# WangYuTum/odometry

Hardware: AMD Instinct MI355X
Metric: tracked frames/sec (1241x376, 4-level pyramid) (higher is better)
Workload: dtype f32

## Files before the change

odometry_amd/csrc/kernels.hip.h:

```cpp
#pragma once
#include <hip/hip_runtime.h>
#include "odo_math.h"

#ifndef ODO_PHASE_STAMPS
#define ODO_PHASE_STAMPS 0
#endif
#if ODO_PHASE_STAMPS
#define ODO_DBG(a) ((a).dbg)
#else
#define ODO_DBG(a) ((unsigned long long*)nullptr)
#endif

#ifndef ODO_KERNEL
#define ODO_KERNEL __global__
#define ODO_KERNEL_T __global__
#endif
#ifdef ODO_LM_CHAIN_TU
#define ODO_DEVICE_VAR static __device__
#else
#define ODO_DEVICE_VAR __device__
#endif

namespace odo {

// ... 425 lines not shown
  }
  for (int x0 = 4; x0 < cols - 4; x0 += 256) {
    const int x = x0 + t;
    float d = 0.0f;
    const bool f = (x < cols - 4) && depth_valid(d = D[x]);
    const unsigned long long bal = __ballot(f);
    const int pre = __popcll(bal & ((1ull << lane) - 1ull));
    if (lane == 0) wave_tot[wv] = __popcll(bal);
    __syncthreads();
    int off = base_sh;
    for (int w = 0; w < wv; w++) off += wave_tot[w];
    if (f) {
      const PointK p = make_point(x, y, d, I[x], k);
      const int i = off + pre;
      pl.a[i] = make_float4(p.X, p.Y, p.Z, p.i1);
      pl.b[i] = make_float4(p.fx_z, p.jw02, p.jw03, p.jw04);
      pl.c[i] = make_float4(p.jw05, p.jw12, p.jw13, p.jw14);
      pl.d[i] = p.jw15;
    }
    __syncthreads();
    if (t == 0) base_sh += (wave_tot[0] + wave_tot[1]) + (wave_tot[2] + wave_tot[3]);
    __syncthreads();
  }
  if (t == 0 && (int)blockIdx.x == kl.row_base[l + 1] - 1) npts[l] = base_sh;
}
ODO_KERNEL void __launch_bounds__(256) kf_fill_kernel(KfLevels kl, float f0, float cx0, float cy0,
                                                      const int* __restrict__ rowcnt, int* __restrict__ npts, PointList pl0, PointList pl1,
                                                      PointList pl2, PointList pl3, PointList pl4, PointList pl5,
                                                      PointList pl6, PointList pl7, int dense_above) {
  const int l = kf_find_level(kl, blockIdx.x);
  const PointList pl = l == 0 ? pl0 : l == 1 ? pl1 : l == 2 ? pl2 : l == 3 ? pl3 : l == 4 ? pl4 : l == 5 ? pl5 : l == 6 ? pl6 : pl7;
  kf_fill_kernel_body<KfLevels>(kl, l, pl, f0, cx0, cy0, rowcnt, npts, dense_above);
}

__device__ __forceinline__ PointK load_point(const PointList& pl, int i) {
  const float4 a = pl.a[i], b = pl.b[i], c = pl.c[i];
  PointK p;
  p.X = a.x; p.Y = a.y; p.Z = a.z; p.i1 = a.w;
  p.fx_z = b.x; p.jw02 = b.y; p.jw03 = b.z; p.jw04 = b.w;
  p.jw05 = c.x; p.jw12 = c.y; p.jw13 = c.z; p.jw14 = c.w;
  p.jw15 = pl.d[i];
  return p;
}

__device__ __forceinline__ const float* lm_uniform_ptr(const float* p) {
  const unsigned long long v = (unsigned long long)p;
  const unsigned lo = (unsigned)__builtin_amdgcn_readfirstlane((int)(v & 0xffffffffu)), hi = (unsigned)__builtin_amdgcn_readfirstlane((int)(v >> 32));
  return (const float*)(((unsigned long long)hi << 32) | lo);
}
__device__ __forceinline__ float ldg_f32(const float* base_uniform, unsigned byte_off) {
  typedef __attribute__((address_space(1))) const char GlobalBytes;
  typedef __attribute__((address_space(1))) const float GlobalFloat;
  return *(GlobalFloat*)((GlobalBytes*)base_uniform + byte_off);
}
template <bool kMayBilinear>
__device__ __forceinline__ bool point_residual_g(const PointK& p, const float* T, const LevelK& k, const float* I2_uniform, int rows,
                                                 int cols, float* r, float J[6]) {
  if (kMayBilinear && k.bilinear) return point_residual<true>(p, T, k, I2_uniform, rows, cols, r, J);
  const float t0 = ((T[0] * p.X + T[4] * p.Y) + T[8] * p.Z) + T[12];
  const float t1 = ((T[1] * p.X + T[5] * p.Y) + T[9] * p.Z) + T[13];
  const float t2 = ((T[2] * p.X + T[6] * p.Y) + T[10] * p.Z) + T[14];
  if (!(t2 > 0.0f)) return false;
  const double t2d = (double)t2, y = rcp_refined_d(t2d);
  const float u = (float)(div_shared_d(k.fl * (double)t0, t2d, y) + (double)k.cx);
  const float v = (float)(div_shared_d(k.fl * (double)t1, t2d, y) + (double)k.cy);
  const float fu = floorf(u), fv = floorf(v);
  if (!(fu < (float)cols) || !(fv < (float)rows) || !(fu >= 0.0f) || !(fv >= 0.0f)) return false;
  const int ui = (int)fu, vi = (int)fv;
  const int px = (ui - 1 >= 0) ? ui - 1 : 0, nx = (ui + 1 < cols) ? ui + 1 : cols - 1;
  const int py = (vi - 1 >= 0) ? vi - 1 : 0, ny = (vi + 1 < rows) ? vi + 1 : rows - 1;
  const unsigned row = (unsigned)vi * (unsigned)cols, ucols = (unsigned)cols;
  const float tc = ldg_f32(I2_uniform, (row + (unsigned)ui) * 4u), tl = ldg_f32(I2_uniform, (row + (unsigned)px) * 4u),
              tr = ldg_f32(I2_uniform, (row + (unsigned)nx) * 4u), tu = ldg_f32(I2_uniform, ((unsigned)py * ucols + (unsigned)ui) * 4u),
              td = ldg_f32(I2_uniform, ((unsigned)ny * ucols + (unsigned)ui) * 4u);
  const float gx = 0.5f * (tr - tl), gy = 0.5f * (td - tu);
  *r = tc - p.i1;
  J[0] = gx * p.fx_z;
  J[1] = gy * p.fx_z;
  J[2] = gx * p.jw02 + gy * p.jw12;
  J[3] = gx * p.jw03 + gy * p.jw13;
  J[4] = gx * p.jw04 + gy * p.jw14;
  J[5] = gx * p.jw05 + gy * p.jw15;
  return true;
}

ODO_KERNEL void __launch_bounds__(kLmBlock) lm_residual_list_kernel(PointList pl, int n, const float* __restrict__ I2, int rows,
                                                                     int cols, LevelK k, const LmState* __restrict__ st,
                                                                     int expect_level, int robust, float huber_delta,
                                                                     const float* __restrict__ scale_sqr_ptr,
                                                                     double* __restrict__ partials) {
  if (!(st->active != 0 && st->level == expect_level)) return;
  float T[16];
#pragma unroll
  for (int i = 0; i < 16; i++) T[i] = st->T[i];
  const float scale_sqr = (robust == 2) ? *scale_sqr_ptr : 1.0f;
  double acc[ODO_NACC];
#pragma unroll
  for (int q = 0; q < ODO_NACC; q++) acc[q] = 0.0;
  for (int idx = blockIdx.x * kLmBlock + threadIdx.x; idx < n; idx += gridDim.x * kLmBlock) {
    const PointK p = load_point(pl, idx);
    float r, J[6];
    if (!point_residual(p, T, k, I2, rows, cols, &r, J)) continue;
    const float w = robust_weight(r, robust, huber_delta, scale_sqr);
    accumulate_row(acc, r, w, J);
  }
  block_reduce_acc(acc, partials + (size_t)blockIdx.x * ODO_NACC);
}

ODO_KERNEL void __launch_bounds__(kLmBlock) lm_residual_only_list_kernel(PointList pl, int n, const float* __restrict__ I2,
                                                                          int rows, int cols, LevelK k,
                                                                          const LmState* __restrict__ st, int expect_level,
                                                                          float* __restrict__ res) {
  if (!(st->active != 0 && st->level == expect_level)) return;
  float T[16];
#pragma unroll
  for (int i = 0; i < 16; i++) T[i] = st->T[i];
  for (int idx = blockIdx.x * kLmBlock + threadIdx.x; idx < n; idx += gridDim.x * kLmBlock) {
    const PointK p = load_point(pl, idx);
    float r = __builtin_nanf(""), rr;
    if (point_residual_only(p, T, k, I2, rows, cols, &rr)) r = rr;
    res[idx] = r;
  }
}

ODO_KERNEL void __launch_bounds__(kLmBlock) lm_residual_only_kernel(LevelView v, LevelK k, const LmState* __restrict__ st,
                                                                     int expect_level, float* __restrict__ res) {
  if (!(st->active != 0 && st->level == expect_level)) return;
  float T[16];
#pragma unroll
  for (int i = 0; i < 16; i++) T[i] = st->T[i];
  const int iw = v.cols - 8, ih = v.rows - 8;
  const int n = (iw > 0 && ih > 0) ? iw * ih : 0;
  for (int idx = blockIdx.x * kLmBlock + threadIdx.x; idx < n; idx += gridDim.x * kLmBlock) {
    const int y = 4 + idx / iw, x = 4 + idx % iw;
    const size_t o = (size_t)y * v.cols + x;
    const float d = v.D1[o];
    float r = __builtin_nanf("");
    if (depth_valid(d)) {
      const PointK p = make_point(x, y, d, v.I1[o], k);
      float rr;
      if (point_residual_only(p, T, k, v.I2, v.rows, v.cols, &rr)) r = rr;
    }
    res[idx] = r;
  }
}

static_assert(sizeof(LmState) <= 64 * sizeof(int), "LmState must fit one wavefront-wide copy");
static_assert(sizeof(LmState) == 64 * sizeof(int), "LmState is exactly 64 dwords");

struct LmTraceRow {
  int level, iter, n_res, accepted, stop;
  float err, lambda_after;
  float delta[6];
};
constexpr int kTraceCap = 128;

__device__ __forceinline__ double readlane_d(double v, int src_lane) {
  const int lo = __builtin_amdgcn_readlane(__double2loint(v), src_lane);
  const int hi = __builtin_amdgcn_readlane(__double2hiint(v), src_lane);
  return __hiloint2double(hi, lo);
}

__device__ __forceinline__ void solve_damped_wave_regs(const double* acc, float lambda, float delta_out[6]) {
  const int lane = threadIdx.x & 63;
  const int i = lane >> 3, j = lane & 7;
  const bool in = (i < 6 && j < 7);
// ... 112 lines not shown
    for (int i = 0; i < 9; i++) {
      const float id = (i == 0 || i == 4 || i == 8) ? 1.0f : 0.0f;
      V[i] = (id + ca * Om[i]) + cb * Om2[i];
    }
  }
  o->tx = (V[0] * a[0] + V[1] * a[1]) + V[2] * a[2];
  o->ty = (V[3] * a[0] + V[4] * a[1]) + V[5] * a[2];
  o->tz = (V[6] * a[0] + V[7] * a[1]) + V[8] * a[2];
}
__device__ __forceinline__ void lm_apply_step_wave(LmState* s, int max_iters) {
  Se3 d;
  se3_exp_wave(s->delta, &d);
  se3_left_update(d, s->cur, &s->inc);
  se3_to_colmajor(s->inc, s->T);
  s->iter++;
  if (!(max_iters > s->iter)) { s->active = 0; s->stop_reason = 3; }
}

constexpr int kRowFloats = 15;
constexpr int kRowSub = 8;
template <int T> struct RowBuf {
  static constexpr int kStride = T / kRowSub + 4;
  static constexpr int W = kRowSub * kStride;
  static constexpr int kBytes = kRowFloats * W * (int)sizeof(float);
};

__device__ __forceinline__ void rows_store(float* __restrict__ rows, int W, int t, const float J[6], float w, float r, bool valid) {
  const int p = (t % kRowSub) * (W / kRowSub) + t / kRowSub;
#pragma unroll
  for (int a = 0; a < 6; a++) {
    rows[a * W + p] = valid ? J[a] : 0.0f;
    rows[(6 + a) * W + p] = valid ? J[a] * w : 0.0f;
  }
  rows[12 * W + p] = valid ? r : 0.0f;
  rows[13 * W + p] = valid ? r * w : 0.0f;
  rows[14 * W + p] = valid ? 1.0f : 0.0f;
}
__device__ __forceinline__ void rows_store_z(float* __restrict__ rows, int W, int t, const float J[6], float w, float r, bool valid) {
  const int p = (t % kRowSub) * (W / kRowSub) + t / kRowSub;
#pragma unroll
  for (int a = 0; a < 6; a++) {
    rows[a * W + p] = J[a];
    rows[(6 + a) * W + p] = J[a] * w;
  }
  rows[12 * W + p] = r;
  rows[13 * W + p] = r * w;
  rows[14 * W + p] = valid ? 1.0f : 0.0f;
}
__device__ __forceinline__ void rows_of_quantity(int q, int* rowA, int* rowB) {
  int a = 0, k = q;
  while (a < 5 && k >= 6 - a) { k -= 6 - a; a++; }
  if (q < 21) { *rowA = 6 + a; *rowB = a + k; }
  else if (q < 27) { *rowA = 6 + (q - 21); *rowB = 12; }
  else if (q == 27) { *rowA = 13; *rowB = 12; }
  else { *rowA = 14; *rowB = 14; }
}
template <int CTRL> __device__ __forceinline__ double dpp_d(double v) {
  const int lo = __builtin_amdgcn_update_dpp(0, __double2loint(v), CTRL, 0xf, 0xf, false);
  const int hi = __builtin_amdgcn_update_dpp(0, __double2hiint(v), CTRL, 0xf, 0xf, false);
  return __hiloint2double(hi, lo);
}
__device__ __forceinline__ double rows_butterfly8(double acc) {
  const double up = dpp_d<0x104>(acc), dn = dpp_d<0x114>(acc);
  acc += (threadIdx.x & 4) ? dn : up;
  acc += dpp_d<0x4E>(acc);
  acc += dpp_d<0xB1>(acc);
  return acc;
}
template <int T, int S>
__device__ __forceinline__ double rows_accumulate(const float* __restrict__ rows, int rowA, int rowB, int s, double acc) {
  static_assert(S == kRowSub && (T / S) % 4 == 0, "the row layout is built for S sub-lanes");
  constexpr int W = RowBuf<T>::W;
  const float4* A = (const float4*)(rows + rowA * W + s * RowBuf<T>::kStride);
  const float4* B = (const float4*)(rows + rowB * W + s * RowBuf<T>::kStride);
#pragma unroll
  for (int i = 0; i < T / S / 4; i++) {
    const float4 a = A[i], b = B[i];
    acc = fma((double)a.x, (double)b.x, acc);
    acc = fma((double)a.y, (double)b.y, acc);
    acc = fma((double)a.z, (double)b.z, acc);
    acc = fma((double)a.w, (double)b.w, acc);
  }
  return acc;
}

__device__ __forceinline__ double wave_sum64(double v) {
  v += dpp_d<0xB1>(v);
  v += dpp_d<0x4E>(v);
  v += dpp_d<0x141>(v);
  v += dpp_d<0x140>(v);
  const double r0 = readlane_d(v, 0), r1 = readlane_d(v, 16), r2 = readlane_d(v, 32), r3 = readlane_d(v, 48);
  return (r0 + r1) + (r2 + r3);
}
__device__ __forceinline__ float tdist_term(float e2, float sigma_sqr) { return e2 * (1.0f + 200.0f) / (200.0f + e2 / sigma_sqr); }
__device__ __forceinline__ float tdist_next_sigma(double total, int n) { return sqrtf((float)(total / (double)n)); }
__device__ __forceinline__ bool tdist_converged(float nxt, float cur) { return !(fabsf(nxt - cur) >= 1e-3f); }
constexpr int kTdistMaxPasses = 1000;

constexpr int kTdistChunksMax = 640;
ODO_KERNEL void __launch_bounds__(1024) lm_tdist_scale_kernel(const float* __restrict__ res, int n,
                                                               const LmState* __restrict__ st, int expect_level,
                                                               float* __restrict__ scale_sqr_out, int list_order,
                                                               int* __restrict__ only_if = nullptr) {
  if (!(st->active != 0 && st->level == expect_level)) return;
  if (only_if) {
    if (__hip_atomic_load(only_if, __ATOMIC_RELAXED, __HIP_MEMORY_SCOPE_AGENT) == 0) return;
    __syncthreads();
    if (threadIdx.x == 0) {
      __hip_atomic_store(only_if, 0, __ATOMIC_RELAXED, __HIP_MEMORY_SCOPE_AGENT);
      only_if[1] += 1;
    }
  }
  __shared__ double shs[1024];
  __shared__ int shn[1024];
  __shared__ float sh_sigma;
  __shared__ int sh_done;
  const int t = threadIdx.x;
  float cur = 5.0f;
  if (list_order) {
    double* part = shs;
    const int lane = t & 63, wv = t >> 6;
    const int nchunk = (n + 63) / 64;
    int n_valid = 0;
    constexpr int kPer = kTdistChunksMax / 16;
    float e2[kPer];
    int cnt = 0;
#pragma unroll
    for (int u = 0; u < kPer; u++) {
      const int c = wv + 16 * u, i = 64 * c + lane;
      const float r = (c < nchunk && i < n) ? res[i] : __builtin_nanf("");
      const bool ok = (r == r);
      e2[u] = ok ? r * r : -1.0f;
      cnt += __popcll(__ballot(ok));
    }
    for (int pass = 0; pass < kTdistMaxPasses; pass++) {
      const float sigma_sqr = cur * cur;
#pragma unroll
      for (int u = 0; u < kPer; u++) {
        const int c = wv + 16 * u;
        if (c < nchunk) {
          const double ws = wave_sum64(e2[u] >= 0.0f ? (double)tdist_term(e2[u], sigma_sqr) : 0.0);
          if (lane == 0) part[c] = ws;
        }
      }
      if (pass == 0 && lane == 0) shn[wv] = cnt;
      __syncthreads();
      if (pass == 0) {
        int tot = 0;
#pragma unroll
        for (int w = 0; w < 16; w++) tot += shn[w];
        n_valid = tot;
      }
      double a = 0.0;
      for (int v = lane; 4 * v < nchunk; v += 64) {
        const int c = 4 * v;
        const double p1 = (c + 1 < nchunk) ? part[c + 1] : 0.0, p2 = (c + 2 < nchunk) ? part[c + 2] : 0.0, p3 = (c + 3 < nchunk) ? part[c + 3] : 0.0;
        a += ((part[c] + p1) + p2) + p3;
      }
      const double total = wave_sum64(a);
      const float nxt = (n_valid > 0) ? tdist_next_sigma(total, n_valid) : cur;
      const bool done = (n_valid == 0) || tdist_converged(nxt, cur);
      cur = nxt;
      if (done) break;
      __syncthreads();
    }
    if (t == 0) *scale_sqr_out = cur * cur;
// ... 489 lines not shown
                                                 const ChainOut chain = ChainOut{nullptr, nullptr, 0, 0, 0, 0, 0, 0, 0, 0}) {
  const int t = threadIdx.x;
  if (t < 64) {
    if (t < (int)(sizeof(LmState) / sizeof(int))) ((int*)st_out)[t] = ((const int*)&s_sh)[t];
    if (final_state && s_sh.finished && t < (int)(sizeof(LmState) / sizeof(int))) ((int*)final_state)[t] = ((const int*)&s_sh)[t];
    if (t == 0) {
      if (s_sh.finished && out) lm_write_result(s_sh, cost_stat, out, done_flag, token, chain);
      if (host_prog) {
        if (s_sh.finished) __hip_atomic_store(host_prog + 1, token, __ATOMIC_RELAXED, __HIP_MEMORY_SCOPE_SYSTEM);
        __hip_atomic_store(host_prog, (token << kProgSeqBits) | (seq + 1), __ATOMIC_RELEASE, __HIP_MEMORY_SCOPE_SYSTEM);
      }
    }
  }
}

__device__ __forceinline__ void lm_step_body(const StepArgs& a, const StepLaunch& q) {
  if (lm_chain_skip(a)) return;
  __builtin_amdgcn_s_setprio(3);
  lm_span_begin(q.span);
  __shared__ LmState s_sh;
  __shared__ double fold_sh[8 * 32];
  __shared__ double acc_sh[32];
  const bool publisher = (blockIdx.x == gridDim.x - 1);
  if (ODO_DBG(a) && publisher && threadIdx.x == 0 && q.seq < 56) ODO_DBG(a)[16 + 2 * q.seq] = wall_clock64();
  lm_fused_prologue(q.st_in, q.part_in, a.lv, a.n_levels, a.lambda0, a.precision, s_sh, fold_sh, acc_sh, a.trace, a.cost_stat,
                    publisher, q.first_of_solve ? a.init : nullptr, a.stop_level);
  const bool run = (s_sh.active != 0 && s_sh.status == 0);
  const int lvl = run ? s_sh.level : 0;
  const StepLevel& L = a.lv[lvl];
  if (run && !publisher && (int)blockIdx.x < L.nblk) {
    __shared__ float rows_sh[kRowFloats * RowBuf<kLmBlock>::W];
    constexpr int kS = 8;
    const int my_q = threadIdx.x / kS, my_s = threadIdx.x % kS;
    int rowA = 0, rowB = 0;
    if (my_q < ODO_NACC) rows_of_quantity(my_q, &rowA, &rowB);
    float T[16];
#pragma unroll
    for (int i = 0; i < 16; i++) T[i] = s_sh.T[i];
    double accq = 0.0;
    const int first = blockIdx.x * kLmBlock;
    for (int base = first; base < L.n; base += L.nblk * kLmBlock) {
      const int idx = base + threadIdx.x;
      float r = 0.0f, w = 0.0f, J[6] = {0.0f, 0.0f, 0.0f, 0.0f, 0.0f, 0.0f};
      bool valid = false;
      if (idx < L.n) {
        const PointK p = load_point(L.pl, idx);
        if (point_residual(p, T, L.k, L.I2, L.rows, L.cols, &r, J)) {
          w = robust_weight(r, a.robust, a.huber_delta, 1.0f);
          valid = true;
        }
      }
      if (base > first) __syncthreads();
      rows_store(rows_sh, RowBuf<kLmBlock>::W, threadIdx.x, J, w, r, valid);
      __syncthreads();
      if (my_q < ODO_NACC) accq = rows_accumulate<kLmBlock, kS>(rows_sh, rowA, rowB, my_s, accq);
    }
    accq = rows_butterfly8(accq);
    if (my_q < ODO_NACC && my_s == 0) q.part_out[(size_t)blockIdx.x * ODO_NACC + my_q] = accq;
  }
  if (publisher) {
    if (threadIdx.x == 0 && run) { s_sh.pending = 1; s_sh.pending_nblk = L.nblk; }
    __syncthreads();
    lm_fused_publish(s_sh, q.st_out, a.host_prog, q.seq, a.token, a.cost_stat, a.out, a.done_flag, a.final_state, chain_out_of(a));
    if (ODO_DBG(a) && threadIdx.x == 0 && q.seq < 56) ODO_DBG(a)[16 + 2 * q.seq + 1] = wall_clock64();
  }
  lm_span_end(q.span);
}

ODO_KERNEL void __launch_bounds__(kLmBlock) lm_step_kernel(StepArgs a) {
  const StepLaunch q = {a.st_in, a.st_out, a.part_in, a.part_out, a.seq, a.first_of_solve, a.span};
  lm_step_body(a, q);
}
ODO_KERNEL void __launch_bounds__(kLmBlock) lm_step_kernel_batch(const StepArgs* __restrict__ table, int seq, int first_of_solve,
                                                                 unsigned long long* span) {
  const StepArgs& a = table[blockIdx.y];
  const StepLaunch q = {a.st2[seq & 1], a.st2[(seq + 1) & 1], a.part2[seq & 1], a.part2[(seq + 1) & 1], seq, first_of_solve, span};
  lm_step_body(a, q);
}

#ifndef ODO_COARSE_BLOCK
#define ODO_COARSE_BLOCK 512
#endif
constexpr int kCoarseBlock = ODO_COARSE_BLOCK;
constexpr int kCoarseLdsBytes = 2 * RowBuf<kLmBlock>::kBytes;
constexpr int kCoarseMaxPoints = 1024;

constexpr int kCoarseRounds = kCoarseMaxPoints / kCoarseBlock;
constexpr int kCoarseChunks = kCoarseRounds * (kCoarseBlock / kWave);
__device__ __forceinline__ float coarse_tdist_sigma(double (*part)[kCoarseChunks], int* cnt, const float e2[kCoarseRounds],
                                                    const bool valid[kCoarseRounds], int nr) {
  constexpr int kW = kCoarseBlock / kWave;
  const int lane = threadIdx.x & 63, wv = threadIdx.x >> 6;
  int my_cnt[kCoarseRounds];
#pragma unroll
  for (int rd = 0; rd < kCoarseRounds; rd++) my_cnt[rd] = __popcll(__ballot(rd < nr && valid[rd]));
  float sigma = 5.0f;
  int n_total = 0;
  for (int pass = 0; pass < kTdistMaxPasses; pass++) {
#pragma unroll
    for (int rd = 0; rd < kCoarseRounds; rd++) {
      const double ws = wave_sum64((rd < nr && valid[rd]) ? (double)tdist_term(e2[rd], sigma * sigma) : 0.0);
      if (lane == 0) { part[pass & 1][rd * kW + wv] = ws; if (pass == 0) cnt[rd * kW + wv] = my_cnt[rd]; }
    }
    __syncthreads();
    if (pass == 0) {
      int tot = 0;
#pragma unroll
      for (int i = 0; i < kCoarseChunks; i++) tot += cnt[i];
      n_total = tot;
    }
    double G = 0.0;
    if (lane < kCoarseChunks / 4) {
      const double* pv = &part[pass & 1][(lane >> 1) * kW + 4 * (lane & 1)];
      G = ((pv[0] + pv[1]) + pv[2]) + pv[3];
    }
    const double total = wave_sum64(G);
    const float nxt = (n_total > 0) ? tdist_next_sigma(total, n_total) : sigma;
    const bool done = (n_total == 0) || tdist_converged(nxt, sigma);
    sigma = nxt;
    if (done) break;
  }
  return sigma;
}
#if ODO_PHASE_STAMPS
ODO_DEVICE_VAR unsigned long long g_lm_diag[24];
#endif
constexpr unsigned long long kArmWaitTicks = 200000000ull;
template <bool kFull, bool kArmed = false>
__device__ __forceinline__ void lm_coarse_body(const StepArgs& a, const StepLaunch& q, int min_level, const unsigned* __restrict__ lv_src) {
#if ODO_PHASE_STAMPS
  const unsigned long long w_entry = (unsigned long long)wall_clock64();
#endif
  if (!kArmed && lm_chain_skip(a)) return;
  __builtin_amdgcn_s_setprio(3);
  lm_span_begin(q.span);
  __shared__ LmState s_sh;
  extern __shared__ __attribute__((aligned(16))) double red_sh[];
  __shared__ double acc_sh[32];
  __shared__ StepLevel lv_sh[ODO_MAX_LEVELS_K];
  __shared__ unsigned long long sm_sh[4];
  unsigned long long arm_g0 = 0;
  if (kArmed && threadIdx.x < 17) arm_g0 = __hip_atomic_load(a.arm + threadIdx.x, __ATOMIC_RELAXED, __HIP_MEMORY_SCOPE_SYSTEM);
  lm_copy_levels(lv_sh, lv_src);
  if (threadIdx.x == 0) {
#pragma unroll
    for (int i = 0; i < 4; i++) sm_sh[i] = 0;
  }
  __shared__ __attribute__((aligned(16))) float arm_pose_sh[16];
  __shared__ __attribute__((aligned(16))) int arm_verdict_sh4[4];
  if (kArmed) {
    if (threadIdx.x < 64) {
      const int lane = (int)threadIdx.x;
      unsigned long long g = arm_g0;
      bool got = __all(lane >= 17 || (int)(g >> 32) == a.token);
      const unsigned long long t0 = (unsigned long long)wall_clock64();
      for (int spin = 0; !got; spin++) {
        if (lane < 17) g = __hip_atomic_load(a.arm + lane, __ATOMIC_RELAXED, __HIP_MEMORY_SCOPE_SYSTEM);
        got = __all(lane >= 17 || (int)(g >> 32) == a.token);
        if (!got && (spin & 15) == 15 && (unsigned long long)wall_clock64() - t0 > (a.fine_wait ? (unsigned long long)a.fine_wait : kArmWaitTicks)) break;
      }
      if (lane < 16) arm_pose_sh[lane] = __uint_as_float((unsigned)g);
      if (lane == 16) arm_verdict_sh4[0] = got ? (int)(unsigned)g : 3;
    }
    __syncthreads();
    if (arm_verdict_sh4[0] == 3) {
      if (threadIdx.x < 64) {
        if (threadIdx.x < (int)(sizeof(LmState) / sizeof(int))) ((int*)&s_sh)[threadIdx.x] = 0;
        if (threadIdx.x == 0) { s_sh.status = -2; s_sh.active = 0; s_sh.finished = 1; }
      }
      __syncthreads();
      lm_fused_publish(s_sh, q.st_out, a.host_prog, q.seq, a.token, a.cost_stat, a.out, a.done_flag, a.final_state);
      return;
    }
    if (arm_verdict_sh4[0] != 1) return;
  } else {
    __syncthreads();
  }
#if ODO_PHASE_STAMPS
  const unsigned long long w_p1 = (unsigned long long)wall_clock64();
#endif
  lm_fused_prologue(q.st_in, q.part_in, lv_sh, a.n_levels, a.lambda0, a.precision, s_sh, red_sh, acc_sh, (kFull ? a.trace : (LmTraceRow*)nullptr), a.cost_stat, true,
                    kArmed ? arm_pose_sh : (q.first_of_solve ? a.init : nullptr), a.stop_level, (!kArmed && a.chain_in_token) ? a.chain_pose : nullptr);
#if ODO_PHASE_STAMPS
  const unsigned long long w_p2 = (unsigned long long)wall_clock64();
#endif
  LmHot hot;
  lm_hot_load(hot, s_sh);
  if (ODO_DBG(a) && threadIdx.x == 0 && q.seq < 56) ODO_DBG(a)[16 + 2 * q.seq] = wall_clock64();
  unsigned long long c_eval = 0, c_red = 0, c_sm = 0, c_it = 0, c_last = ODO_DBG(a) ? __builtin_readcyclecounter() : 0;
  const unsigned long long c_begin = c_last, w_begin = ODO_DBG(a) ? (unsigned long long)wall_clock64() : 0;
  auto lap = [&](unsigned long long& sum) {
    if (ODO_DBG(a)) { const unsigned long long now = __builtin_readcyclecounter(); sum += now - c_last; c_last = now; }
  };
  static_assert(kCoarseBlock == 2 * kLmBlock, "two 256-point virtual blocks per round");
  constexpr int kS = 8;
  constexpr int kVbMax = (kCoarseMaxPoints + kLmBlock - 1) / kLmBlock;
  __shared__ double part_sh[kVbMax][32];
  __shared__ double sc_part[2][kCoarseChunks];
  __shared__ int sc_cnt[kCoarseChunks];
  const int tl = threadIdx.x & (kLmBlock - 1), half = threadIdx.x >> 8;
  float* rows_sh = (float*)red_sh + half * (kRowFloats * RowBuf<kLmBlock>::W);
  const int my_q = tl / kS, my_s = tl % kS;
  int rowA = 0, rowB = 0;
  if (my_q < ODO_NACC) rows_of_quantity(my_q, &rowA, &rowB);
  PointK cpt[kCoarseRounds];
  bool cpt_ok[kCoarseRounds] = {false, false};
  int cpt_level = -1;
  for (int guard = 0; guard < 4096; guard++) {
    const bool run = (s_sh.active != 0 && s_sh.status == 0 && s_sh.level >= min_level);
    if (!run) break;
    c_it++;
    const StepLevel& L = lv_sh[s_sh.level];
    const float* I2u = lm_uniform_ptr(L.I2);
    float T[16];
#pragma unroll
    for (int i = 0; i < 16; i++) T[i] = s_sh.T[i];
    const int nvb = L.nblk;
    if (s_sh.level != cpt_level) {
      cpt_level = s_sh.level;
#pragma unroll
      for (int rd = 0; rd < kCoarseRounds; rd++) {
        const int vb = 2 * rd + half, idx = vb * kLmBlock + tl;
        cpt_ok[rd] = vb < nvb && idx < L.n;
        if (cpt_ok[rd]) cpt[rd] = load_point(L.pl, idx);
      }
    }
    float td_r[kCoarseRounds] = {0.0f, 0.0f}, td_J[kCoarseRounds][6] = {{0.0f, 0.0f, 0.0f, 0.0f, 0.0f, 0.0f}, {0.0f, 0.0f, 0.0f, 0.0f, 0.0f, 0.0f}};
    bool td_valid[kCoarseRounds] = {false, false};
    float td_scale_sqr = 1.0f;
    if ((kFull && a.robust == 2)) {
      float e2[kCoarseRounds];
#pragma unroll
      for (int rd = 0; rd < kCoarseRounds; rd++) {
        if (cpt_ok[rd]) td_valid[rd] = point_residual_g<kFull>(cpt[rd], T, L.k, I2u, L.rows, L.cols, &td_r[rd], td_J[rd]);
        e2[rd] = td_r[rd] * td_r[rd];
      }
      const float sg = coarse_tdist_sigma(sc_part, sc_cnt, e2, td_valid, (nvb + 1) / 2);
      td_scale_sqr = sg * sg;
    }
#pragma unroll
    for (int vb0 = 0; vb0 < 2 * kCoarseRounds; vb0 += 2) {
      if (vb0 >= nvb) break;
      const int vb = vb0 + half;
      float r = 0.0f, w = 0.0f, J[6] = {0.0f, 0.0f, 0.0f, 0.0f, 0.0f, 0.0f};
      bool valid = false;
      if ((kFull && a.robust == 2)) {
        r = td_r[vb0 / 2]; valid = td_valid[vb0 / 2];
#pragma unroll
        for (int i = 0; i < 6; i++) J[i] = td_J[vb0 / 2][i];
        if (valid) w = robust_weight(r, 2, a.huber_delta, td_scale_sqr);
      } else if (cpt_ok[vb0 / 2]) {
        if (point_residual_g<kFull>(cpt[vb0 / 2], T, L.k, I2u, L.rows, L.cols, &r, J)) {
          w = robust_weight(r, kFull ? a.robust : (a.robust == 1 ? 1 : 0), a.huber_delta, 1.0f);
          valid = true;
        }
      }
      if (vb0 > 0) __syncthreads();
      rows_store_z(rows_sh, RowBuf<kLmBlock>::W, tl, J, w, r, valid);
      __syncthreads();
      if (vb0 == 0) lap(c_eval);
      double accq = 0.0;
      if (vb < nvb) {
        if (my_q < ODO_NACC) accq = rows_accumulate<kLmBlock, kS>(rows_sh, rowA, rowB, my_s, accq);
        accq = rows_butterfly8(accq);
      }
      if (nvb == 1) {
        if (half == 0 && my_q < ODO_NACC && my_s == 0) {
          double v = 0.0;
          v += accq;
          double acc = 0.0;
          acc += v;
#pragma unroll
          for (int g = 1; g < 8; g++) acc += 0.0;
          acc_sh[my_q] = acc;
        }
      } else if (vb < nvb && my_q < ODO_NACC && my_s == 0) {
        part_sh[vb][my_q] = accq;
      }
    }
    __syncthreads();
    if (nvb > 1) {
      const int fq = threadIdx.x & 31, fseg = threadIdx.x >> 5;
      double* fold_sh = red_sh;
      if (fseg < 8) {
        double v = 0.0;
        if (fq < ODO_NACC)
          for (int b = fseg; b < nvb; b += 8) v += part_sh[b][fq];
        fold_sh[fseg * 32 + fq] = v;
      }
      __syncthreads();
      if (threadIdx.x < ODO_NACC) {
        double acc = 0.0;
#pragma unroll
        for (int g = 0; g < 8; g++) acc += fold_sh[g * 32 + threadIdx.x];
        acc_sh[threadIdx.x] = acc;
      }
    }
    lap(c_red);
    lm_state_machine_hot(hot, lv_sh, a.n_levels, a.lambda0, a.precision, s_sh, acc_sh, (kFull ? a.trace : (LmTraceRow*)nullptr), a.cost_stat, true,
                         ODO_DBG(a) ? sm_sh : nullptr, a.stop_level);
    lap(c_sm);
  }
#if ODO_PHASE_STAMPS
  const unsigned long long w_loop_end = (unsigned long long)wall_clock64();
#endif
  if (threadIdx.x == 0) lm_hot_store(hot, s_sh);
  lm_fused_publish(s_sh, q.st_out, a.host_prog, q.seq, a.token, a.cost_stat, a.out, a.done_flag, a.final_state, chain_out_of(a));
#if ODO_PHASE_STAMPS
  if (ODO_DBG(a) && threadIdx.x == 0) {
    const unsigned long long now = (unsigned long long)wall_clock64();
    g_lm_diag[4] += w_begin - w_entry; g_lm_diag[5] += w_loop_end - w_begin; g_lm_diag[6] += now - w_loop_end;
    g_lm_diag[16] += w_p1 - w_entry; g_lm_diag[17] += w_p2 - w_p1; g_lm_diag[18] += w_begin - w_p2;
    if (g_lm_diag[1] && w_entry > g_lm_diag[1] && w_entry - g_lm_diag[1] < 100000ull) { g_lm_diag[7] += w_entry - g_lm_diag[1]; g_lm_diag[3] += w_entry - g_lm_diag[2]; g_lm_diag[14] += 1; }
    g_lm_diag[0] = now; g_lm_diag[8] += 1;
  }
#endif
  if (ODO_DBG(a) && threadIdx.x == 0) {
    if (q.seq < 56) ODO_DBG(a)[16 + 2 * q.seq + 1] = wall_clock64();
    ODO_DBG(a)[0] += c_eval; ODO_DBG(a)[1] += c_red; ODO_DBG(a)[2] += c_sm; ODO_DBG(a)[3] += c_it;
    ODO_DBG(a)[4] += __builtin_readcyclecounter() - c_begin; ODO_DBG(a)[5] += 1;
    ODO_DBG(a)[6] += (unsigned long long)wall_clock64() - w_begin;
#pragma unroll
    for (int i = 0; i < 4; i++) ODO_DBG(a)[8 + i] += sm_sh[i];
  }
  lm_span_end(q.span);
}

#ifdef ODO_LM_CHAIN_TU
static __global__ void __launch_bounds__(kCoarseBlock) lm_coarse_kernel(StepArgs a, int min_level) {
  const StepLaunch q = {a.st_in, a.st_out, a.part_in, a.part_out, a.seq, a.first_of_solve, a.span};
  lm_coarse_body<false>(a, q, min_level, lm_kernarg_words());
}
static __global__ void __launch_bounds__(kCoarseBlock) lm_coarse_armed_kernel(StepArgs a, int min_level) {
  const StepLaunch q = {a.st_in, a.st_out, a.part_in, a.part_out, a.seq, a.first_of_solve, a.span};
  lm_coarse_body<false, true>(a, q, min_level, lm_kernarg_words());
}
static __global__ void __launch_bounds__(kCoarseBlock) lm_coarse_full_kernel(StepArgs a, int min_level) {
  const StepLaunch q = {a.st_in, a.st_out, a.part_in, a.part_out, a.seq, a.first_of_solve, a.span};
  lm_coarse_body<true>(a, q, min_level, lm_kernarg_words());
}
#endif
template <bool kFull>
__device__ __forceinline__ void lm_coarse_batch_entry(const StepArgs* __restrict__ table, int seq, int first_of_solve, unsigned long long* span) {
// ... 1309 lines not shown
```

odometry_amd/csrc/odometry_hip.hip:

```cpp
#include <hip/hip_runtime.h>
#include <hip/hip_ext.h>
#include <stdarg.h>
#include <stdio.h>
#include <stdlib.h>
#include <string.h>
#include <chrono>

#include <atomic>
#include <mutex>
#include <new>
#include <thread>
#include <utility>
#include <vector>

#include "../../include/odometry_hip.h"
#include "kernels.hip.h"

using namespace odo;

static thread_local char g_err[512] = "";
static int fail(const char* fmt, ...) {
  va_list ap;
  va_start(ap, fmt);
  vsnprintf(g_err, sizeof(g_err), fmt, ap);
// ... 663 lines not shown
  int ev_phase;
  long ev_solves;
  std::vector<hipEvent_t>* ev_pool;
  double ev_total_us, ev_bytes, ev_coarse_us;
  long ev_launches, ev_active, ev_coarse_launches;
  long ev_sampled, ev_coarse_all;
  unsigned long long* d_span;
  int span_used;
  struct SpanTag { unsigned char coarse; long solve; int idx; };
  std::vector<SpanTag>* span_kind;
  double ev_period_us, ev_cperiod_us;
  long ev_period_n, ev_cperiod_n;
  int last_coarse;
  int last_coarse_batch;
  int trace_stale;
  int record;
  unsigned reset_gen;
  float* h_res; float* d_res_map; int* h_done; int* d_done; int token;
  int coarse;
  int fine_k;
  int fine_bails;
  int fine_k_cfg;
  int fine_k_last;
  int fine_strikes;
  int fine_clean;
  int fine_offs;
  unsigned fine_wait;
  unsigned fine_epoch;
  int fine_fault;
  int fine_home;
  unsigned long long* d_xbuf;
  int fused;
  int mode;
  int bilinear;
  unsigned* dispatch_words;
  int dense_plain_div;
  void (*idle_pump)(void*);
  void* idle_arg;
  float* h_out;
  LmTraceRow* h_trace;
  float* h_cost;
  int last_evals, last_launches;
  double last_bytes;
  int iters[ODO_MAX_LEVELS];
  int launches_level[ODO_MAX_LEVELS];
  LmJob job;
  LmJob chained;
  LmJob armed;
  int arm_on;
  unsigned long long* h_arm; unsigned long long* d_arm_map;
  long arm_used, arm_aborted;
  long arm_fault_at; unsigned arm_wait;
  float* d_chain_pose;
  int* d_chain_guard;
  float kf_rule[7];
  int kf_on;
  int slot_next;
  int last_token, last_slot;
};

static inline LevelK lm_level_k(const odo_lm* m, int level) {
  LevelK k = make_level_k(m->K.f0, m->K.cx0, m->K.cy0, level);
  k.bilinear = m->bilinear;
  return k;
}

extern "C" int odo_lm_create(odo_ctx* ctx, float lambda, float precision, const int* max_iters, int n_levels,
                             const float init_colmajor[16], int robust, float huber_delta, const odo_intrinsics* K,
                             odo_lm** out) {
  if (!ctx || !out || !max_iters || !init_colmajor) return fail("odo_lm_create: NULL arg");
  *out = nullptr;
  if (n_levels < 1 || n_levels > ODO_MAX_LEVELS) return fail("odo_lm_create: n_levels %d out of range", n_levels);
  if (robust < 0 || robust > 2) return fail("odo_lm_create: robust must be 0, 1 or 2");
  odo_lm* m = new (std::nothrow) odo_lm();
  if (!m) return fail("out of memory");
  memset(m, 0, sizeof(*m));
  m->ctx = ctx; m->lambda = lambda; m->precision = precision; m->huber_delta = huber_delta;
  m->n_levels = n_levels; m->robust = robust;
  for (int i = 0; i < n_levels; i++) m->max_iters[i] = max_iters[i];
  m->K = K ? *K : kKitti00;
  memcpy(m->init, init_colmajor, sizeof(m->init));
  HIP_OK(hipSetDevice(ctx->device));
  HIP_OK(lm_chain_setup());
  HIP_OK(hipGetSymbolAddress((void**)&m->dispatch_words, HIP_SYMBOL(g_lm_fine_dispatch)));
  HIP_OK(hipMalloc((void**)&m->d_state, sizeof(LmState) * 3));
  m->ust = m->d_state; m->upo = 0;
  m->fuse_dense_max = getenv("ODO_FUSE_DENSE_MAX") ? atoi(getenv("ODO_FUSE_DENSE_MAX")) : 131072;
  HIP_OK(hipMalloc((void**)&m->d_partials, sizeof(double) * 2 * kLmMaxBlocks * ODO_NACC));
  HIP_OK(hipMalloc((void**)&m->d_init, sizeof(float) * 16));
  HIP_OK(hipMalloc((void**)&m->d_out, sizeof(float) * 48));
  HIP_OK(hipMalloc((void**)&m->d_trace, sizeof(LmTraceRow) * kTraceCap));
  m->d_cost = m->d_out + 26;
  HIP_OK(hipMalloc((void**)&m->d_scale, sizeof(float)));
  HIP_OK(hipMalloc((void**)&m->d_ts_xbuf, sizeof(unsigned long long) * kTsXbufWords));
  HIP_OK(hipMemset(m->d_ts_xbuf, 0, sizeof(unsigned long long) * kTsXbufWords));
  HIP_OK(hipMalloc((void**)&m->d_ts_gave_up, 2 * sizeof(int)));
  HIP_OK(hipMemset(m->d_ts_gave_up, 0, 2 * sizeof(int)));
  m->ts_epoch = 0;
  m->ts_multi = getenv("ODO_TDIST_SINGLE") ? 0 : 1;
  m->fine_passes = getenv("ODO_LM_FINE_PASSES") ? atoi(getenv("ODO_LM_FINE_PASSES")) : 2;
  m->ts_fault = getenv("ODO_TDIST_MULTI_FAULT") ? 1 : 0;
  m->ts_wait = getenv("ODO_LM_FINE_WAIT_US") ? (unsigned)(100L * atol(getenv("ODO_LM_FINE_WAIT_US"))) : 0u;
  HIP_OK(hipHostMalloc((void**)&m->h_out, sizeof(float) * 48, hipHostMallocDefault));
  HIP_OK(hipHostMalloc((void**)&m->h_trace, sizeof(LmTraceRow) * kTraceCap, hipHostMallocDefault));
  m->h_cost = m->h_out + 26;
  HIP_OK(hipHostMalloc((void**)&m->h_res, sizeof(float) * 48 * 2, hipHostMallocMapped | hipHostMallocCoherent));
  memset(m->h_res, 0, sizeof(float) * 48 * 2);
  HIP_OK(hipMalloc((void**)&m->d_chain_pose, sizeof(float) * 32));
  HIP_OK(hipMemset(m->d_chain_pose, 0, sizeof(float) * 32));
  m->d_chain_guard = (int*)(m->d_chain_pose + 16);
  HIP_OK(hipHostGetDevicePointer((void**)&m->d_res_map, m->h_res, 0));
  HIP_OK(hipHostMalloc((void**)&m->h_done, sizeof(int) * 4, hipHostMallocMapped | hipHostMallocCoherent));
  HIP_OK(hipHostGetDevicePointer((void**)&m->d_done, m->h_done, 0));
  m->h_done[0] = 0; m->h_done[1] = 0;
  HIP_OK(hipHostMalloc((void**)&m->h_prog, sizeof(int) * 32, hipHostMallocMapped | hipHostMallocCoherent));
  HIP_OK(hipHostGetDevicePointer((void**)&m->d_prog, m->h_prog, 0));
  memset(m->h_prog, 0, sizeof(int) * 32);
  HIP_OK(hipMalloc((void**)&m->d_npts, sizeof(int) * ODO_MAX_LEVELS));
  HIP_OK(hipHostMalloc((void**)&m->h_npts, sizeof(int) * ODO_MAX_LEVELS, hipHostMallocMapped | hipHostMallocCoherent));
  HIP_OK(hipHostGetDevicePointer((void**)&m->hm_npts, m->h_npts, 0));
  for (LmCandSet& cs : m->cand) {
    HIP_OK(hipMalloc((void**)&cs.d_npts, sizeof(int) * ODO_MAX_LEVELS));
    HIP_OK(hipHostMalloc((void**)&cs.h_npts, sizeof(int) * ODO_MAX_LEVELS, hipHostMallocMapped | hipHostMallocCoherent));
    HIP_OK(hipHostGetDevicePointer((void**)&cs.hm_npts, cs.h_npts, 0));
    cs.tag = -1;
  }
  m->ahead.active = 0;
  HIP_OK(hipEventCreateWithFlags(&m->ahead.ev, hipEventDisableTiming));
  m->record = 1;
  m->mode = getenv("ODO_LM_MODE") ? atoi(getenv("ODO_LM_MODE")) : 0;
  m->dense_plain_div = getenv("ODO_DENSE_PLAIN_DIV") ? 1 : 0;
  m->fused = getenv("ODO_LM_UNFUSED") ? 0 : 1;
  m->coarse = getenv("ODO_LM_NO_COARSE") ? 0 : 1;
  m->fine_k = getenv("ODO_LM_NO_FINE") ? 0 : (getenv("ODO_LM_FINE_K") ? atoi(getenv("ODO_LM_FINE_K")) : 32);
  if (m->fine_k < 0 || m->fine_k > kFineKMax) m->fine_k = 32;
  m->fine_k_cfg = m->fine_k;
  m->fine_fault = getenv("ODO_LM_FINE_FAULT") ? 1 : 0;
  m->fine_home = next_home_xcd(ctx->device);
  m->fine_wait = getenv("ODO_LM_FINE_WAIT_US") ? (unsigned)(100L * atol(getenv("ODO_LM_FINE_WAIT_US"))) : 0u;
  HIP_OK(hipMalloc((void**)&m->d_xbuf, sizeof(unsigned long long) * kFineXbufWords));
  HIP_OK(hipMemset(m->d_xbuf, 0, sizeof(unsigned long long) * kFineXbufWords));
  m->poll = getenv("ODO_NO_POLL") ? 0 : 1;
  m->run_ahead = getenv("ODO_RUN_AHEAD") ? atoi(getenv("ODO_RUN_AHEAD")) : 2;
  HIP_OK(hipMemsetAsync(m->d_trace, 0, sizeof(LmTraceRow) * kTraceCap, ctx->stream));
  memset(m->h_trace, 0, sizeof(LmTraceRow) * kTraceCap);
  memset(m->h_out, 0, sizeof(float) * 48);
  *out = m;
  return 0;
}

static void lm_arm_abort(odo_lm* m);
extern "C" int odo_lm_destroy(odo_lm* m) {
  if (!m) return 0;
  lm_arm_abort(m);
  if (m->ahead.ev) { (void)hipEventSynchronize(m->ahead.ev); (void)hipEventDestroy(m->ahead.ev); }
  (void)hipStreamSynchronize(m->ctx->stream);
  void* dv[] = {m->d_state, m->d_partials, m->d_xbuf, m->d_init, m->d_out, m->d_trace, m->d_scale, m->d_res, m->d_chain_pose, m->d_ts_xbuf, m->d_ts_gave_up,
                m->d_rowcnt, m->d_npts, m->cand[0].d_rowcnt, m->cand[0].d_npts, m->cand[1].d_rowcnt, m->cand[1].d_npts};
  for (void* q : dv) if (q) (void)hipFree(q);
  for (int l = 0; l < ODO_MAX_LEVELS; l++) {
    void* pv[] = {m->pl[l].a, m->pl[l].b, m->pl[l].c, m->pl[l].d, m->cand[0].pl[l].a, m->cand[0].pl[l].b, m->cand[0].pl[l].c, m->cand[0].pl[l].d,
                  m->cand[1].pl[l].a, m->cand[1].pl[l].b, m->cand[1].pl[l].c, m->cand[1].pl[l].d};
    for (void* q : pv) if (q) (void)hipFree(q);
  }
  (void)hipHostFree(m->h_npts);
  (void)hipHostFree(m->cand[0].h_npts);
// ... 2078 lines not shown
```

Before: 4093.

## Process both coarse LM rounds at once with doubled row buffers

In the coarse LM kernel, when more than two virtual blocks are present, both rounds of points are now evaluated together. A paired residual routine issues all ten image gathers before using any of them, and each round writes to its own LDS row buffer, so one barrier and one fused dual-accumulator pass replace the former serialized two-pass loop. Dynamic LDS is doubled and the max dynamic shared size attribute is set on the coarse kernels. The armed path's span-begin is also moved so it is only recorded once the verdict is known. The larger LDS footprint may reduce occupancy.

```diff
diff --git a/odometry_amd/csrc/kernels.hip.h b/odometry_amd/csrc/kernels.hip.h
--- a/odometry_amd/csrc/kernels.hip.h
+++ b/odometry_amd/csrc/kernels.hip.h
@@ -531,6 +531,48 @@
   J[4] = gx * p.jw04 + gy * p.jw14;
   J[5] = gx * p.jw05 + gy * p.jw15;
   return true;
+}
+__device__ __forceinline__ void point_residual_g_pair(const PointK (&p)[2], const bool (&have)[2], const float* T, const LevelK& k,
+                                                      const float* I2_uniform, int rows, int cols, float (&r)[2], float (&J)[2][6],
+                                                      bool (&valid)[2]) {
+  const unsigned ucols = (unsigned)cols;
+  unsigned o_c[2], o_l[2], o_r[2], o_u[2], o_d[2];
+#pragma unroll
+  for (int c = 0; c < 2; c++) {
+    const float t0 = ((T[0] * p[c].X + T[4] * p[c].Y) + T[8] * p[c].Z) + T[12];
+    const float t1 = ((T[1] * p[c].X + T[5] * p[c].Y) + T[9] * p[c].Z) + T[13];
+    const float t2 = ((T[2] * p[c].X + T[6] * p[c].Y) + T[10] * p[c].Z) + T[14];
+    const double t2d = (double)t2, y = rcp_refined_d(t2d);
+    const float u = (float)(div_shared_d(k.fl * (double)t0, t2d, y) + (double)k.cx);
+    const float v = (float)(div_shared_d(k.fl * (double)t1, t2d, y) + (double)k.cy);
+    const float fu = floorf(u), fv = floorf(v);
+    const bool ok = have[c] & (t2 > 0.0f) & (fu < (float)cols) & (fv < (float)rows) & (fu >= 0.0f) & (fv >= 0.0f);
+    const int ui = (int)(ok ? fu : 0.0f), vi = (int)(ok ? fv : 0.0f);
+    const int px = (ui - 1 >= 0) ? ui - 1 : 0, nx = (ui + 1 < cols) ? ui + 1 : cols - 1;
+    const int py = (vi - 1 >= 0) ? vi - 1 : 0, ny = (vi + 1 < rows) ? vi + 1 : rows - 1;
+    const unsigned row = (unsigned)vi * ucols;
+    o_c[c] = (row + (unsigned)ui) * 4u; o_l[c] = (row + (unsigned)px) * 4u; o_r[c] = (row + (unsigned)nx) * 4u;
+    o_u[c] = ((unsigned)py * ucols + (unsigned)ui) * 4u; o_d[c] = ((unsigned)ny * ucols + (unsigned)ui) * 4u;
+    valid[c] = ok;
+  }
+  float tc[2], tl[2], tr[2], tu[2], td[2];
+#pragma unroll
+  for (int c = 0; c < 2; c++) {
+    tc[c] = ldg_f32(I2_uniform, o_c[c]); tl[c] = ldg_f32(I2_uniform, o_l[c]); tr[c] = ldg_f32(I2_uniform, o_r[c]);
+    tu[c] = ldg_f32(I2_uniform, o_u[c]); td[c] = ldg_f32(I2_uniform, o_d[c]);
+  }
+#pragma unroll
+  for (int c = 0; c < 2; c++) {
+    const float gx = 0.5f * (tr[c] - tl[c]), gy = 0.5f * (td[c] - tu[c]);
+    const bool ok = valid[c];
+    r[c] = ok ? tc[c] - p[c].i1 : 0.0f;
+    J[c][0] = ok ? gx * p[c].fx_z : 0.0f;
+    J[c][1] = ok ? gy * p[c].fx_z : 0.0f;
+    J[c][2] = ok ? gx * p[c].jw02 + gy * p[c].jw12 : 0.0f;
+    J[c][3] = ok ? gx * p[c].jw03 + gy * p[c].jw13 : 0.0f;
+    J[c][4] = ok ? gx * p[c].jw04 + gy * p[c].jw14 : 0.0f;
+    J[c][5] = ok ? gx * p[c].jw05 + gy * p[c].jw15 : 0.0f;
+  }
 }
 
 ODO_KERNEL void __launch_bounds__(kLmBlock) lm_residual_list_kernel(PointList pl, int n, const float* __restrict__ I2, int rows,
@@ -809,6 +851,28 @@
     acc = fma((double)a.w, (double)b.w, acc);
   }
   return acc;
+}
+template <int T, int S>
+__device__ __forceinline__ void rows_accumulate2(const float* __restrict__ rows0, const float* __restrict__ rows1, int rowA, int rowB, int s,
+                                                 double& acc0, double& acc1) {
+  static_assert(S == kRowSub && (T / S) % 4 == 0, "the row layout is built for S sub-lanes");
+  constexpr int W = RowBuf<T>::W;
+  const float4* A0 = (const float4*)(rows0 + rowA * W + s * RowBuf<T>::kStride);
+  const float4* B0 = (const float4*)(rows0 + rowB * W + s * RowBuf<T>::kStride);
+  const float4* A1 = (const float4*)(rows1 + rowA * W + s * RowBuf<T>::kStride);
+  const float4* B1 = (const float4*)(rows1 + rowB * W + s * RowBuf<T>::kStride);
+#pragma unroll
+  for (int i = 0; i < T / S / 4; i++) {
+    const float4 a0 = A0[i], b0 = B0[i], a1 = A1[i], b1 = B1[i];
+    acc0 = fma((double)a0.x, (double)b0.x, acc0);
+    acc1 = fma((double)a1.x, (double)b1.x, acc1);
+    acc0 = fma((double)a0.y, (double)b0.y, acc0);
+    acc1 = fma((double)a1.y, (double)b1.y, acc1);
+    acc0 = fma((double)a0.z, (double)b0.z, acc0);
+    acc1 = fma((double)a1.z, (double)b1.z, acc1);
+    acc0 = fma((double)a0.w, (double)b0.w, acc0);
+    acc1 = fma((double)a1.w, (double)b1.w, acc1);
+  }
 }
 
 __device__ __forceinline__ double wave_sum64(double v) {
@@ -1464,7 +1528,7 @@
 #define ODO_COARSE_BLOCK 512
 #endif
 constexpr int kCoarseBlock = ODO_COARSE_BLOCK;
-constexpr int kCoarseLdsBytes = 2 * RowBuf<kLmBlock>::kBytes;
+constexpr int kCoarseLdsBytes = 4 * RowBuf<kLmBlock>::kBytes;
 constexpr int kCoarseMaxPoints = 1024;
 
 constexpr int kCoarseRounds = kCoarseMaxPoints / kCoarseBlock;
@@ -1515,7 +1579,7 @@
 #endif
   if (!kArmed && lm_chain_skip(a)) return;
   __builtin_amdgcn_s_setprio(3);
-  lm_span_begin(q.span);
+  if (!kArmed) lm_span_begin(q.span);
   __shared__ LmState s_sh;
   extern __shared__ __attribute__((aligned(16))) double red_sh[];
   __shared__ double acc_sh[32];
@@ -1545,6 +1609,7 @@
       if (lane == 16) arm_verdict_sh4[0] = got ? (int)(unsigned)g : 3;
     }
     __syncthreads();
+    if (arm_verdict_sh4[0] == 1 || arm_verdict_sh4[0] == 3) lm_span_begin(q.span);
     if (arm_verdict_sh4[0] == 3) {
       if (threadIdx.x < 64) {
         if (threadIdx.x < (int)(sizeof(LmState) / sizeof(int))) ((int*)&s_sh)[threadIdx.x] = 0;
@@ -1552,6 +1617,7 @@
       }
       __syncthreads();
       lm_fused_publish(s_sh, q.st_out, a.host_prog, q.seq, a.token, a.cost_stat, a.out, a.done_flag, a.final_state);
+      lm_span_end(q.span);
       return;
     }
     if (arm_verdict_sh4[0] != 1) return;
@@ -1575,6 +1641,7 @@
     if (ODO_DBG(a)) { const unsigned long long now = __builtin_readcyclecounter(); sum += now - c_last; c_last = now; }
   };
   static_assert(kCoarseBlock == 2 * kLmBlock, "two 256-point virtual blocks per round");
+  static_assert(kCoarseRounds == 2 && kCoarseLdsBytes >= 2 * kCoarseRounds * RowBuf<kLmBlock>::kBytes, "a row buffer per virtual block");
   constexpr int kS = 8;
   constexpr int kVbMax = (kCoarseMaxPoints + kLmBlock - 1) / kLmBlock;
   __shared__ double part_sh[kVbMax][32];
@@ -1582,10 +1649,11 @@
   __shared__ int sc_cnt[kCoarseChunks];
   const int tl = threadIdx.x & (kLmBlock - 1), half = threadIdx.x >> 8;
   float* rows_sh = (float*)red_sh + half * (kRowFloats * RowBuf<kLmBlock>::W);
+  float* rows_sh1 = rows_sh + 2 * (kRowFloats * RowBuf<kLmBlock>::W);
   const int my_q = tl / kS, my_s = tl % kS;
   int rowA = 0, rowB = 0;
   if (my_q < ODO_NACC) rows_of_quantity(my_q, &rowA, &rowB);
-  PointK cpt[kCoarseRounds];
+  PointK cpt[kCoarseRounds] = {};
   bool cpt_ok[kCoarseRounds] = {false, false};
   int cpt_level = -1;
   for (int guard = 0; guard < 4096; guard++) {
@@ -1607,40 +1675,66 @@
         if (cpt_ok[rd]) cpt[rd] = load_point(L.pl, idx);
       }
     }
-    float td_r[kCoarseRounds] = {0.0f, 0.0f}, td_J[kCoarseRounds][6] = {{0.0f, 0.0f, 0.0f, 0.0f, 0.0f, 0.0f}, {0.0f, 0.0f, 0.0f, 0.0f, 0.0f, 0.0f}};
-    bool td_valid[kCoarseRounds] = {false, false};
-    float td_scale_sqr = 1.0f;
-    if ((kFull && a.robust == 2)) {
-      float e2[kCoarseRounds];
-#pragma unroll
-      for (int rd = 0; rd < kCoarseRounds; rd++) {
-        if (cpt_ok[rd]) td_valid[rd] = point_residual_g<kFull>(cpt[rd], T, L.k, I2u, L.rows, L.cols, &td_r[rd], td_J[rd]);
-        e2[rd] = td_r[rd] * td_r[rd];
-      }
-      const float sg = coarse_tdist_sigma(sc_part, sc_cnt, e2, td_valid, (nvb + 1) / 2);
-      td_scale_sqr = sg * sg;
-    }
-#pragma unroll
-    for (int vb0 = 0; vb0 < 2 * kCoarseRounds; vb0 += 2) {
-      if (vb0 >= nvb) break;
-      const int vb = vb0 + half;
+    const bool tdist = kFull && a.robust == 2;
+    if (nvb > 2) {
+      float r[kCoarseRounds] = {0.0f, 0.0f}, w[kCoarseRounds] = {0.0f, 0.0f};
+      float J[kCoarseRounds][6] = {{0.0f, 0.0f, 0.0f, 0.0f, 0.0f, 0.0f}, {0.0f, 0.0f, 0.0f, 0.0f, 0.0f, 0.0f}};
+      bool valid[kCoarseRounds] = {false, false};
+      if (!(kFull && L.k.bilinear)) {
+        point_residual_g_pair(cpt, cpt_ok, T, L.k, I2u, L.rows, L.cols, r, J, valid);
+      } else {
+#pragma unroll
+        for (int rd = 0; rd < kCoarseRounds; rd++)
+          if (cpt_ok[rd]) valid[rd] = point_residual_g<kFull>(cpt[rd], T, L.k, I2u, L.rows, L.cols, &r[rd], J[rd]);
+      }
+      float td_scale_sqr = 1.0f;
+      if (tdist) {
+        const float e2[kCoarseRounds] = {r[0] * r[0], r[1] * r[1]};
+        const float sg = coarse_tdist_sigma(sc_part, sc_cnt, e2, valid, kCoarseRounds);
+        td_scale_sqr = sg * sg;
+      }
+#pragma unroll
+      for (int rd = 0; rd < kCoarseRounds; rd++)
+        if (valid[rd]) w[rd] = robust_weight(r[rd], kFull ? a.robust : (a.robust == 1 ? 1 : 0), a.huber_delta, td_scale_sqr);
+      rows_store_z(rows_sh, RowBuf<kLmBlock>::W, tl, J[0], w[0], r[0], valid[0]);
+      rows_store_z(rows_sh1, RowBuf<kLmBlock>::W, tl, J[1], w[1], r[1], valid[1]);
+      __syncthreads();
+      lap(c_eval);
+      double acc0 = 0.0, acc1 = 0.0;
+      if (my_q < ODO_NACC) rows_accumulate2<kLmBlock, kS>(rows_sh, rows_sh1, rowA, rowB, my_s, acc0, acc1);
+      acc0 = rows_butterfly8(acc0);
+      acc1 = rows_butterfly8(acc1);
+      if (my_q < ODO_NACC && my_s == 0) {
+        part_sh[half][my_q] = acc0;
+        if (2 + half < nvb) part_sh[2 + half][my_q] = acc1;
+      }
+    } else {
+      float td_r[kCoarseRounds] = {0.0f, 0.0f}, td_J[6] = {0.0f, 0.0f, 0.0f, 0.0f, 0.0f, 0.0f};
+      bool td_valid[kCoarseRounds] = {false, false};
+      float td_scale_sqr = 1.0f;
+      if (tdist) {
+        if (cpt_ok[0]) td_valid[0] = point_residual_g<kFull>(cpt[0], T, L.k, I2u, L.rows, L.cols, &td_r[0], td_J);
+        const float e2[kCoarseRounds] = {td_r[0] * td_r[0], 0.0f};
+        const float sg = coarse_tdist_sigma(sc_part, sc_cnt, e2, td_valid, 1);
+        td_scale_sqr = sg * sg;
+      }
+      const int vb = half;
       float r = 0.0f, w = 0.0f, J[6] = {0.0f, 0.0f, 0.0f, 0.0f, 0.0f, 0.0f};
       bool valid = false;
-      if ((kFull && a.robust == 2)) {
-        r = td_r[vb0 / 2]; valid = td_valid[vb0 / 2];
-#pragma unroll
-        for (int i = 0; i < 6; i++) J[i] = td_J[vb0 / 2][i];
+      if (tdist) {
+        r = td_r[0]; valid = td_valid[0];
+#pragma unroll
+        for (int i = 0; i < 6; i++) J[i] = td_J[i];
         if (valid) w = robust_weight(r, 2, a.huber_delta, td_scale_sqr);
-      } else if (cpt_ok[vb0 / 2]) {
-        if (point_residual_g<kFull>(cpt[vb0 / 2], T, L.k, I2u, L.rows, L.cols, &r, J)) {
+      } else if (cpt_ok[0]) {
+        if (point_residual_g<kFull>(cpt[0], T, L.k, I2u, L.rows, L.cols, &r, J)) {
           w = robust_weight(r, kFull ? a.robust : (a.robust == 1 ? 1 : 0), a.huber_delta, 1.0f);
           valid = true;
         }
       }
-      if (vb0 > 0) __syncthreads();
       rows_store_z(rows_sh, RowBuf<kLmBlock>::W, tl, J, w, r, valid);
       __syncthreads();
-      if (vb0 == 0) lap(c_eval);
+      lap(c_eval);
       double accq = 0.0;
       if (vb < nvb) {
         if (my_q < ODO_NACC) accq = rows_accumulate<kLmBlock, kS>(rows_sh, rowA, rowB, my_s, accq);
diff --git a/odometry_amd/csrc/odometry_hip.hip b/odometry_amd/csrc/odometry_hip.hip
--- a/odometry_amd/csrc/odometry_hip.hip
+++ b/odometry_amd/csrc/odometry_hip.hip
@@ -769,6 +769,8 @@
   memcpy(m->init, init_colmajor, sizeof(m->init));
   HIP_OK(hipSetDevice(ctx->device));
   HIP_OK(lm_chain_setup());
+  HIP_OK(hipFuncSetAttribute((const void*)lm_coarse_kernel_batch, hipFuncAttributeMaxDynamicSharedMemorySize, kCoarseLdsBytes));
+  HIP_OK(hipFuncSetAttribute((const void*)lm_coarse_full_kernel_batch, hipFuncAttributeMaxDynamicSharedMemorySize, kCoarseLdsBytes));
   HIP_OK(hipGetSymbolAddress((void**)&m->dispatch_words, HIP_SYMBOL(g_lm_fine_dispatch)));
   HIP_OK(hipMalloc((void**)&m->d_state, sizeof(LmState) * 3));
   m->ust = m->d_state; m->upo = 0;
```

Measured after the change: 4076. Within noise of the previous version (-0.4%).
